# rongzhao-zhang/EfficientQ

Measured on AMD Instinct MI355X. Metric: ptq_calibration_throughput, higher is better.
Workload: dtype i8xi8->i32 (exact) for the Gram systems and per-iteration loss convs of the layers with quantised input, f32/f64 elsewhere

## Files before the change

### efficientq_amd/_lib.py

```python
from __future__ import annotations

import ctypes as C
import os

import torch

_HERE = os.path.dirname(os.path.abspath(__file__))
LIB_PATH = os.path.join(_HERE, "libeffq_hip.so")

EFFQ_OK = 0
_ERR_NAMES = {1: "EFFQ_ERR_ARG", 2: "EFFQ_ERR_HIP", 3: "EFFQ_ERR_WORKSPACE", 4: "EFFQ_ERR_NO_DEVICE",
              5: "EFFQ_ERR_NOT_CONVERGED"}


class EffqError(RuntimeError):
    pass


class Geom(C.Structure):
    _fields_ = [(n, C.c_int32) for n in
                ("N", "C1", "C2", "D", "H", "W", "KD", "KH", "KW", "SD", "SH", "SW", "PD", "PH", "PW")]

    def out_dims(self):
        return ((self.D + 2 * self.PD - self.KD) // self.SD + 1,
# ... 27 lines not shown
                ("ainv_pool", C.c_void_p), ("n_ainv", C.c_int32),
                ("prox_ws", C.c_void_p), ("prox_ws_bytes", C.c_size_t),
                ("red_ws", C.c_void_p),
                ("fp_ws", C.c_void_p), ("fp_ws_bytes", C.c_size_t),
                ("fp_pred", C.c_void_p), ("fp_traj_ws", C.c_void_p), ("fp_traj_ws_bytes", C.c_size_t),
                ("inv_ws", C.c_void_p), ("inv_ws_bytes", C.c_size_t),
                ("inv_ws_side", C.c_void_p), ("inv_ws_side_bytes", C.c_size_t),
                ("conv_ws", C.c_void_p), ("conv_ws_bytes", C.c_size_t),
                ("stream_main", C.c_void_p), ("stream_loss", C.c_void_p), ("stream_side", C.c_void_p),
                ("stream_side2", C.c_void_p), ("inv_ws_side2", C.c_void_p), ("inv_ws_side2_bytes", C.c_size_t),
                ("loss_Au", C.c_void_p), ("loss_Bu", C.c_void_p), ("loss_syy", C.c_void_p),
                ("loss_planes", C.c_void_p), ("loss_nplanes", C.c_int32), ("res_ring", C.c_void_p),
                ("channel_wise", C.c_int32), ("alpha_ring", C.c_void_p), ("w_iters_ring", C.c_void_p)]


class ProfRecord(C.Structure):
    _fields_ = [("kind", C.c_int32), ("iter", C.c_int32), ("loss_kind", C.c_int32), ("c2", C.c_int32), ("n", C.c_int32),
                ("geom", Geom), ("ms", C.c_float)]


SIGNATURES = {
    "effq_last_error": (C.c_char_p, []),
    "effq_version": (_I, []),
    "effq_device_count": (_I, [C.POINTER(C.c_int)]),
    "effq_quant_dequant_f32": (_I, [_P, _P, _F, _F, _I, _P, _P, _SZ, _P]),
    "effq_quant_dequant_f64path": (_I, [_P, _P, _D, _D, _I, _P, _P, _P, _SZ, _P]),
    "effq_reduce_ws_bytes": (_SZ, []),
    "effq_abs_sum_f64": (_I, [_P, _SZ, _P, _P, _P]),
    "effq_moments_f64": (_I, [_P, _SZ, _P, _P, _P]),
    "effq_alpha_stats_f64": (_I, [_P, _P, _D, _D, _I, _SZ, _P, _P, _P, _P]),
    "effq_fp_init": (_I, [_P, _P, _P]),
    "effq_fp_update": (_I, [_P, _D, _I, _P]),
    "effq_alpha_fixed_point": (_I, [_P, _SZ, _I, _D, _D, _D, _I, _I, _P, _P, _P]),
    "effq_fp_small_max": (_SZ, []),
    "effq_fixed_point_small": (_I, [_P, _P, _P, _SZ, _I, _D, _D, _D, _I, _P, _P]),
    "effq_fp_coop_max": (_SZ, []),
    "effq_fp_coop_set_spin_limit": (_I, [C.c_uint]),
    "effq_fixed_point_coop": (_I, [_P, _P, _P, _SZ, _I, _D, _D, _D, _I, _P, _P, _P]),
    "effq_fp_bucket_max": (_SZ, []),
    "effq_fp_bucket_ws_bytes": (_SZ, [_SZ]),
    "effq_fixed_point_bucket": (_I, [_P, _P, _P, _SZ, _I, _D, _D, _D, _I, _P, _P, _SZ, _P]),
    "effq_fp_bracket_ws_bytes": (_SZ, [_SZ]),
    "effq_fp_bracket_init": (_I, [_P, _P, _SZ, _I, _I, _P, _SZ, _P]),
    "effq_fp_bracket_run": (_I, [_P, _SZ, _I, _D, _D, _D, _I, _I, _P, _P, _P]),
    "effq_fp_bracket_stats": (_I, [_P, _SZ, _I, _D, _D, _P, _P, _P]),
    "effq_fp_bracket_update": (_I, [_SZ, _I, _D, _D, _D, _I, _P, _P, _P]),
    "effq_fp_traj_max": (_SZ, []),
    "effq_fp_traj_ws_bytes": (_SZ, [_SZ]),
    "effq_spd_inverse_prepare": (_I, [_P]),
    "effq_fp_traj_pred_bytes": (_SZ, []),
    "effq_fixed_point_traj": (_I, [_P, _P, _P, _SZ, _I, _D, _D, _D, _I, _P, _P, _P, _SZ, _P]),
    "effq_fixed_point_bucket_rec": (_I, [_P, _P, _P, _SZ, _I, _D, _D, _D, _I, _P, _P, _SZ, _P, _P]),
    "effq_fixed_point_coop_rec": (_I, [_P, _P, _P, _SZ, _I, _D, _D, _D, _I, _P, _P, _P, _P]),
    "effq_fp_check": (_I, [_P, _P, _P]),
    "effq_fp_channels_max_row": (_I, []),
    "effq_fixed_point_channels": (_I, [_P, _P, _P, _I, _I, _I, _D, _I, _P, _P, _P, _P]),
    "effq_fixed_point_channels_proj": (_I, [_P, _P, _P, _I, _I, _I, _D, _I, _P, _P, _P, _P, _F, _P, _P, _P, _I, _I, _D,
                                            _D, _P]),
    "effq_gram_packed_elems": (_SZ, [_I, _I]),
    "effq_gram_pack": (_I, [_P, _P, _I, _I, _P, _P]),
    "effq_gram_unpack": (_I, [_P, _I, _I, _P, _P, _P]),
    "effq_act_quant_backward": (_I, [_P, _P, _I, _P, _P, _P, _SZ, _P, _P]),
    "effq_att_classes_ws_bytes": (_SZ, []),
    "effq_att_classes": (_I, [_P, _LL, _P, _P, _P, C.POINTER(C.c_int32), _P, _P]),
    "effq_prof_enable": (_I, [_I]),
    "effq_prof_count": (_I, []),
    "effq_prof_read": (_I, [_I, C.POINTER(ProfRecord)]),
    "effq_admm_num_inverses": (_I, [_D, _D, _I, _I]),
    "effq_admm_run": (_I, [C.POINTER(AdmmRunArgs)]),
    "effq_admm_select_best": (_I, [_P, _I, _P, _P, _SZ, _SZ, _P, _P, _P, _P]),
    "effq_gram_ws_bytes": (_SZ, [_GP, _I]),
    "effq_gram_accum": (_I, [_P, _P, _P, _GP, _I, _P, _P, _I, _P, _SZ, _P]),
    "effq_gram_plan_query": (_I, [_GP, _I, _IP, _IP, _IP, _IP, _LLP, _IP, _IP]),
    "effq_gram_i8_supported": (_I, [_GP, _I]),
    "effq_gram_i8_ws_bytes": (_SZ, [_GP, _I]),
    "effq_gram_accum_i8": (_I, [_P, _P, _GP, _I, _P, _I, _P, _P, _P, _I, _LL, _P, _P, _I, _P, _SZ, _P]),
    "effq_gram_accum_i8_unw": (_I, [_P, _P, _GP, _I, _P, _I, _P, _P, _P, _I, _LL, _P, _P, _I, _P, _P, _P, _SZ, _P]),
    "effq_gram_i8_plan_query": (_I, [_GP, _I, _LL, _IP, _IP, _IP, _IP, _IP, _IP]),
    "effq_upsample_trilinear": (_I, [_P, _I, _I, _I, _I, _I, _I, _I, _I, _P, _P]),
    "effq_gram_f64_supported": (_I, [_GP, _I]),
    "effq_gram_f64_ws_bytes": (_SZ, [_GP, _I]),
    "effq_gram_f64": (_I, [_P, _P, _GP, _I, _P, _P, _P, _SZ, _P]),
    "effq_gram_f64_plan_query": (_I, [_GP, _I, _IP, _IP, _IP, _IP]),
    "effq_gram_loss_ws_bytes": (_SZ, [_I]),
    "effq_gram_loss": (_I, [_P, _P, _P, _P, _P, _I, _I, _I, _P, _P, _SZ, _P]),
    "effq_packed_bytes": (_SZ, [_SZ, _I]),
    "effq_pack_levels": (_I, [_P, _SZ, _I, _P, _P]),
    "effq_unpack_levels": (_I, [_P, _SZ, _I, _P, _P]),
    "effq_ainv_ld": (_I, [_I]),
    "effq_fp_bracket_export_words": (_SZ, []),
    "effq_fp_bracket_export": (_I, [_P, _SZ, _P, _P, _SZ, _P]),
    "effq_fp_bracket_rebase": (_I, [_P, _P, _SZ, _P]),
    "effq_fp_bracket_import": (_I, [_P, _SZ, _P, _I, _SZ, _P, _P, _SZ, _P]),
    "effq_admm_uses_traj": (_I, [_SZ, _I]),
    "effq_gram_loss_i8_supported": (_I, [_I, _I, _I, _I]),
    "effq_gram_loss_i8_num_planes": (_I, [C.c_longlong]),
    "effq_gram_loss_i8_planes_bytes": (_SZ, [_I, _I, _I]),
    "effq_gram_loss_i8_prepare": (_I, [_P, _I, _I, _P, _I, _I, _P, _P, _P]),
    "effq_gram_loss_i8_ws_bytes": (_SZ, []),
    "effq_gram_loss_i8": (_I, [_P, _I, _P, _P, _P, _P, _P, _P, _P, _I, _I, _I, _I, _I, _I, _P, _P, _SZ, _P]),
    "effq_spd_inverse_ws_bytes": (_SZ, [_I]),
    "effq_spd_inverse": (_I, [_P, _I, _I, _D, _D, _P, _P, _SZ, _P]),
    "effq_spd_inverse_plan": (_I, [_I, _IP, _IP, _IP]),
    "effq_prox_plan_query": (_I, [_I, _I, _IP, _IP, _IP, _IP]),
    "effq_prox_ws_bytes": (_SZ, [_I, _I]),
    "effq_prox_solve": (_I, [_P, _P, _P, _P, _P, _P, _I, _I, _I, _D, _D, _P, _P, _P, _SZ, _P]),
    "effq_prox_solve_shifted": (_I, [_P, _P, _P, _P, _P, _P, _I, _I, _I, _D, _D, _D, _I, _P, _P, _P, _SZ, _P]),
    "effq_admm_presum": (_I, [_P, _P, _P, _SZ, _P]),
    "effq_admm_project_dual": (_I, [_P, _P, _P, _I, _P, _P, _F, _P, _SZ, _P]),
    "effq_conv_plan_query": (_I, [_GP, _I, _IP, _IP, _IP, _IP, _IP, _IP, _IP, _IP, _LLP]),
    "effq_conv_i8_plan_query": (_I, [_GP, _I, _IP, _IP, _IP, _IP]),
    "effq_conv_i8s_plan_query": (_I, [_GP, _I, _I, _IP, _IP, _IP, _IP, _IP, _IP, _IP]),
    "effq_conv_i8_supported": (_I, [_GP, _I, _I]),
    "effq_conv_i8s_supported": (_I, [_GP, _I, _I]),
    "effq_conv_i8s_ws_bytes": (_SZ, [_GP, _I, _I]),
    "conv3d_calib_step_i8s": (_I, [_P, _P, _P, _P, _GP, _P, _I, _P, _I, _I, _P, _P, _SZ, _P]),
    "effq_conv_i8_ws_bytes": (_SZ, [_GP]),
    "conv3d_calib_step_i8": (_I, [_P, _P, _P, _P, _GP, _P, _I, _P, _I, _P, _P, _SZ, _P]),
    "effq_conv_i8_out_supported": (_I, [_GP, _I, _I]),
    "conv3d_quant_forward_i8": (_I, [_P, _P, _P, _P, _P, _GP, _P, _I, _P, _I, _P, _P, _P, _SZ, _P]),
    "effq_conv_ws_bytes": (_SZ, [_GP]),
    "conv3d_quant_calib_step": (_I, [_P, _P, _P, _P, _P, _GP, _P, _I, _P, _P, _P, _SZ, _P]),
    "effq_adam_step": (_I, [_P, _P, _P, _P, _D, _D, _D, _D, _I, _SZ, _P]),
    "effq_window_gather": (_I, [_P, _I, _I, _I, _I, _I, _I, _I, _I, _I, _I, _I, _I, _I, _I, _P, _P]),
    "effq_window_put": (_I, [_P, _I, _I, _I, _I, _I, _I, _I, _P, _P]),
    "effq_window_stitch": (_I, [_P, _I, _I, _I, _I, _I, _I, _I, _I, _I, _I, _I, _P, _P, _P, _I, _P, _P]),
    "effq_seg_tallies": (_I, [_P, _P, _I, _LL, _I, _I, _F, _P, _P, _SZ, _P]),
    "effq_seg_sweep": (_I, [_P, _P, _I, _LL, _I, _I, _F, _P, _P]),
    "effq_seg_sweep_edges": (_I, [_I, _F, _P]),
    "effq_seg_sweep_plan": (_I, [_I, _LL, _I, _IP, _IP]),
    "effq_seg_labels": (_I, [_P, _I, _I, _LL, _I, _I, _F, _I, _P, _P]),
    "effq_seg_labels_source": (_I, [_P, _I, _P, _P, _P, _P, _P, _I, _I, _F, _P, _P]),
    "effq_seg_probs_source": (_I, [_P, _I, _P, _P, _P, _P, _P, _I, _P, _P, _P]),
    "effq_seg_agreement": (_I, [_P, _P, _I, _LL, _I, _I, _F, _P, _P, _P, _P, _P, _SZ, _P]),
    "effq_cc_ws_bytes": (_SZ, [_I, _I, _I, _I]),
    "effq_cc_label": (_I, [_P, _I, _I, _I, _I, _I, _P, _P, _P, _SZ, _P]),
    "effq_seg_lesions": (_I, [_P, _P, _I, _I, _I, _I, _I, _I, _F, _I, _P, _P, _SZ, _P]),
    "effq_cc_table_ws_bytes": (_SZ, [_I, _I, _I, _I, _I]),
    "effq_cc_table": (_I, [_P, _I, _I, _I, _I, _I, _I, _P, _P, _P, _SZ, _P]),
    "effq_seg_lesion_table": (_I, [_P, _P, _I, _I, _I, _I, _I, _I, _F, _I, _I, _P, _P, _P, _P, _SZ, _P]),
    "effq_label_clean_ws_bytes": (_SZ, [_I, _I, _I]),
    "effq_label_clean": (_I, [_P, _I, _I, _I, _I, _I, _P, _P, _P, _P, _P, _SZ, _P]),
    "effq_label_tallies_ws_bytes": (_SZ, []),
    "effq_label_tallies": (_I, [_P, _P, _I, _I, _LL, _P, _P, _P, _SZ, _P]),
    "effq_surf_ws_bytes": (_SZ, [_I, _I, _I, _I]),
    "effq_edt_sq": (_I, [_P, _I, _I, _I, _I, _P, _P, _SZ, _P]),
    "effq_seg_surface": (_I, [_P, _P, _I, _I, _I, _I, _I, _I, _F, _P, _P, _P, _SZ, _P]),
    "effq_surf_mm_ws_bytes": (_SZ, [_I, _I, _I, _I]),
    "effq_edt_sq_mm": (_I, [_P, _I, _I, _I, _I, _F, _F, _F, _P, _P, _SZ, _P]),
    "effq_seg_surface_mm": (_I, [_P, _P, _I, _I, _I, _I, _I, _I, _F, _F, _F, _F, _P, _P, _P, _P, _SZ, _P]),
    "effq_prep_window": (_I, [_P, _SZ, _F, _F, _P]),
    "effq_prep_resample": (_I, [_P, _I, _I, _I, _I, _D, _D, _D, _I, _P, _I, _I, _I, _P]),
    "effq_prep_bbox_moments": (_I, [_P, _I, _I, _I, _I, _I, _P, _P, _P, _P, _SZ, _P]),
    "effq_prep_sqdev": (_I, [_P, _I, _LL, _I, _P, _P, _P, _SZ, _P]),
    "effq_prep_standardise_crop": (_I, [_P, _I, _I, _I, _I, _I, _P, _P, _P, _P, _P, _P]),
    "effq_prep_crop_u8": (_I, [_P, _I, _I, _I, _I, _P, _P, _P, _P]),
    "effq_prep_union_mask": (_I, [_P, _I, _LL, _I, _P, _P]),
    "effq_prep_reorient": (_I, [_P, _I, _I, _I, _I, _P, _I, _I, _P, _P]),
    "effq_prep_reorient_plan": (_I, [_P, _I, _I, _P]),
}

SEG_TALLIES_WS_BYTES = 1024 * 3 * 8 * 4
SEG_TALLIES_MAX_CLASSES = 8
SEG_AGREEMENT_WS_BYTES = 768 * (4 * SEG_TALLIES_MAX_CLASSES * 8 + (3 * SEG_TALLIES_MAX_CLASSES + 1) * 4)
SEG_ARGMAX, SEG_SIGMOID = 0, 1
SEG_SWEEP_BINS = 4096
# ... 37 lines not shown
```

### efficientq_amd/csrc/gram_f64.hip

```cpp
#include "common.h"

namespace effq {

typedef double f64x4g __attribute__((ext_vector_type(4)));

constexpr int GF_VC = 32;
constexpr int GF_T = 256;
constexpr int GF_MAXN = 128, GF_MAXC2 = 64;
constexpr int GF_MAXTILES = 72;

struct GramF64Params {
  const float* x;
  const float* y;
  effq_geom g;
  int n, has_bias, np, c2p, ld;
  int od, oh, ow;
  long long V;
  int nchunk, ntiles, te, tc;
  double* slab;
};

template <int TPW>
__global__ __launch_bounds__(GF_T, (TPW <= 6) ? 4 : 2) void k_gram_f64(GramF64Params p) {
  extern __shared__ __attribute__((aligned(16))) double rows[];
  __shared__ int tab_a[GF_MAXTILES], tab_b[GF_MAXTILES];
  const int tid = threadIdx.x, lane = tid & 63, wid = tid >> 6;
  const int lr = lane & 15, lk = lane >> 4;
  if (tid == 0) {
    int t = 0;
    for (int i = 0; i < p.te; ++i)
      for (int j = i; j < p.te; ++j) {
        tab_a[t] = 16 * i;
        tab_b[t] = 16 * j;
        ++t;
      }
    for (int c = 0; c < p.tc; ++c)
      for (int j = 0; j < p.te; ++j) {
        tab_a[t] = p.np + 16 * c;
        tab_b[t] = 16 * j;
        ++t;
      }
  }
  __syncthreads();
  int aoff[TPW], boff[TPW];
  f64x4g acc[TPW];
#pragma unroll
  for (int t = 0; t < TPW; ++t) {
    const int tile = wid + 4 * t;
    const bool ok = tile < p.ntiles;
    aoff[t] = ok ? tab_a[tile] : 0;
    boff[t] = ok ? tab_b[tile] : 0;
#pragma unroll
    for (int r = 0; r < 4; ++r) acc[t][r] = 0.0;
  }
  const int nw = p.n - p.has_bias;
  __shared__ int qtab[GF_MAXN];
  __shared__ int vrow[GF_VC][4];
  {
    const int k3 = p.g.KD * p.g.KH * p.g.KW, k2 = p.g.KH * p.g.KW;
    for (int q = tid; q < nw; q += GF_T) {
      const int c = q / k3, kr = q - c * k3;
      const int kd = kr / k2, kr2 = kr - kd * k2;
      const int kh = kr2 / p.g.KW, kw = kr2 - kh * p.g.KW;
      qtab[q] = c | (kd << 16) | (kh << 20) | (kw << 24);
    }
  }
  const int rowlen = p.np + p.c2p;
  const int V = (int)p.V;
  for (int ch = blockIdx.x; ch < p.nchunk; ch += gridDim.x) {
    __syncthreads();
    const int v0 = ch * GF_VC;
    if (tid < GF_VC) {
      const int v = v0 + tid;
      int t = v;
      const int ow_ = t % p.ow;
      t /= p.ow;
      const int oh_ = t % p.oh;
      t /= p.oh;
      const int od_ = t % p.od;
      vrow[tid][0] = (v < V) ? t / p.od : -1;
      vrow[tid][1] = od_ * p.g.SD - p.g.PD;
      vrow[tid][2] = oh_ * p.g.SH - p.g.PH;
      vrow[tid][3] = ow_ * p.g.SW - p.g.PW;
    }
    __syncthreads();
    for (int e = tid; e < GF_VC * rowlen; e += GF_T) {
      const int vl = e / rowlen, q = e - vl * rowlen;
      const int nn = vrow[vl][0];
      double val = 0.0;
      if (nn >= 0) {
        if (q < nw) {
          const int pk = qtab[q];
          const int c = pk & 0xffff;
          const int id = vrow[vl][1] + ((pk >> 16) & 15), ih = vrow[vl][2] + ((pk >> 20) & 15),
                    iw = vrow[vl][3] + ((pk >> 24) & 15);
          if (id >= 0 && id < p.g.D && ih >= 0 && ih < p.g.H && iw >= 0 && iw < p.g.W)
            val = (double)p.x[((((size_t)nn * p.g.D + id) * p.g.H + ih) * p.g.W + iw) * p.g.C1 + c];
        } else if (q < p.n) {
          val = 1.0;
        } else if (q >= p.np && q - p.np < p.g.C2) {
          val = (double)p.y[(size_t)(v0 + vl) * p.g.C2 + (q - p.np)];
        }
      }
      rows[vl * p.ld + q] = val;
    }
    __syncthreads();
#pragma unroll 2
    for (int ks = 0; ks < GF_VC / 4; ++ks) {
      const double* r0 = rows + (ks * 4 + lk) * p.ld + lr;
#pragma unroll
      for (int t = 0; t < TPW; ++t) {
        const double a = r0[aoff[t]], b = r0[boff[t]];
        acc[t] = __builtin_amdgcn_mfma_f64_16x16x4f64(a, b, acc[t], 0, 0, 0);
      }
    }
  }
#pragma unroll
  for (int t = 0; t < TPW; ++t) {
    const int tile = wid + 4 * t;
    if (tile < p.ntiles) {
      double* dst = p.slab + ((size_t)blockIdx.x * p.ntiles + tile) * 256;
#pragma unroll
      for (int r = 0; r < 4; ++r) dst[r * 64 + lane] = acc[t][r];
    }
  }
}

__global__ __launch_bounds__(256) void k_gram_f64_reduce(GramF64Params p, int nslab, double* __restrict__ Au,
                                                         double* __restrict__ Bu) {
  const int tile = blockIdx.x, e = threadIdx.x;
  double s = 0.0;
  for (int w = 0; w < nslab; ++w) s += p.slab[((size_t)w * p.ntiles + tile) * 256 + e];
  const int r = e >> 6, lane = e & 63;
  const int row = (lane >> 4) + 4 * r, col = lane & 15;
  const int nau = p.te * (p.te + 1) / 2;
  if (tile < nau) {
    int i = 0, rem = tile;
    while (rem >= p.te - i) {
      rem -= p.te - i;
      ++i;
    }
    const int j = i + rem;
    const int gi = 16 * i + row, gj = 16 * j + col;
    if (gi < p.n && gj < p.n) {
      Au[(size_t)gi * p.n + gj] = s;
      if (i != j) Au[(size_t)gj * p.n + gi] = s;
    }
  } else {
    const int t = tile - nau;
    const int c = t / p.te, j = t - c * p.te;
    const int gc = 16 * c + row, gj = 16 * j + col;
    if (gc < p.g.C2 && gj < p.n) Bu[(size_t)gc * p.n + gj] = s;
  }
}

static bool gram_f64_plan(const effq_geom* g, int has_bias, GramF64Params* p) {
  if (g == nullptr) return false;
  const long long nw = (long long)g->C1 * g->KD * g->KH * g->KW;
  const long long n = nw + (has_bias ? 1 : 0);
  if (n < 1 || n > GF_MAXN || g->C2 < 1 || g->C2 > GF_MAXC2) return false;
  const int od = (g->D + 2 * g->PD - g->KD) / g->SD + 1, oh = (g->H + 2 * g->PH - g->KH) / g->SH + 1,
            ow = (g->W + 2 * g->PW - g->KW) / g->SW + 1;
  if (od <= 0 || oh <= 0 || ow <= 0 || g->N <= 0) return false;
  p->g = *g;
  p->n = (int)n;
  p->has_bias = has_bias ? 1 : 0;
  p->np = ((int)n + 15) / 16 * 16;
  p->c2p = (g->C2 + 15) / 16 * 16;
  p->ld = p->np + p->c2p + 2;
  p->od = od; p->oh = oh; p->ow = ow;
  p->V = (long long)g->N * od * oh * ow;
  p->nchunk = (int)((p->V + GF_VC - 1) / GF_VC);
  p->te = p->np / 16;
  p->tc = p->c2p / 16;
  p->ntiles = p->te * (p->te + 1) / 2 + p->tc * p->te;
  return p->ntiles <= GF_MAXTILES && p->V < ((long long)1 << 31) - GF_VC && g->KD <= 15 && g->KH <= 15 && g->KW <= 15;
}

static int gram_f64_grid(const GramF64Params& p) { return p.nchunk < 1024 ? p.nchunk : 1024; }

static int gram_f64_tpw(const GramF64Params& p) {
  const int tpw = (p.ntiles + 3) / 4;
  return tpw <= 3 ? 3 : (tpw <= 6 ? 6 : (tpw <= 11 ? 11 : 18));
}

}
using namespace effq;

extern "C" {

int effq_gram_f64_supported(const effq_geom* g, int has_bias) {
  GramF64Params p;
  return gram_f64_plan(g, has_bias, &p) ? 1 : 0;
}

size_t effq_gram_f64_ws_bytes(const effq_geom* g, int has_bias) {
  GramF64Params p;
  if (!gram_f64_plan(g, has_bias, &p)) return 0;
  return (size_t)gram_f64_grid(p) * p.ntiles * 256 * sizeof(double);
}

int effq_gram_f64(const float* x_ndhwc, const float* y_ndhwc, const effq_geom* g, int has_bias, double* Au, double* Bu,
                  void* ws, size_t ws_bytes, void* stream) {
  EFFQ_CHECK_ARG(x_ndhwc && y_ndhwc && g && Au && Bu && ws);
  GramF64Params p;
  if (!gram_f64_plan(g, has_bias, &p)) {
    set_error("gram_f64: unsupported geometry (n = C1*k^3 + bias <= %d, C2 <= %d)", GF_MAXN, GF_MAXC2);
    return EFFQ_ERR_ARG;
  }
  const size_t need = effq_gram_f64_ws_bytes(g, has_bias);
  if (ws_bytes < need) {
    set_error("gram_f64: workspace %zu < required %zu", ws_bytes, need);
    return EFFQ_ERR_WORKSPACE;
  }
  p.x = x_ndhwc;
  p.y = y_ndhwc;
  p.slab = reinterpret_cast<double*>(ws);
  const int grid = gram_f64_grid(p);
  const size_t lds = (size_t)GF_VC * p.ld * sizeof(double);
  hipStream_t st = as_stream(stream);
#define EFFQ_GF(TPW_) hipLaunchKernelGGL((k_gram_f64<TPW_>), dim3(grid), dim3(GF_T), lds, st, p)
  switch (gram_f64_tpw(p)) {
    case 3: EFFQ_GF(3); break;
    case 6: EFFQ_GF(6); break;
    case 11: EFFQ_GF(11); break;
    default: EFFQ_GF(18); break;
  }
#undef EFFQ_GF
  EFFQ_LAUNCH_CHECK();
  hipLaunchKernelGGL(k_gram_f64_reduce, dim3(p.ntiles), dim3(256), 0, st, p, grid, Au, Bu);
  EFFQ_LAUNCH_CHECK();
  return EFFQ_OK;
}

int effq_gram_f64_plan_query(const effq_geom* g, int has_bias, int* nchunk, int* grid, int* ntiles, int* tpw) {
  EFFQ_CHECK_ARG(g && nchunk && grid && ntiles && tpw);
  GramF64Params p;
  EFFQ_CHECK_ARG(gram_f64_plan(g, has_bias, &p));
  *nchunk = p.nchunk;
  *grid = gram_f64_grid(p);
  *ntiles = p.ntiles;
  *tpw = gram_f64_tpw(p);
  return EFFQ_OK;
}

}
```

### efficientq_amd/hip_ops.py

```python
from __future__ import annotations

import ctypes as C
import math
from typing import Optional, Tuple

import torch

from . import _lib
from ._lib import Geom, check

ADMM_TOL = 1e-5
FP_BRACKET_MIN = 1 << 18
DP_GATHER_AFTER = 4
DP_GATHER_MAX_BYTES = 128 << 20


def _ptr(t: Optional[torch.Tensor]):
    return None if t is None else C.c_void_p(t.data_ptr())


def to_ndhwc(x: torch.Tensor) -> torch.Tensor:
    return x.permute(0, 2, 3, 4, 1).contiguous()


# ... 379 lines not shown
        check(self.lib.effq_gram_plan_query(C.byref(geom), int(has_bias), C.byref(vec), C.byref(nb), C.byref(npairs),
                                            C.byref(nsplit), C.byref(vps), C.byref(fold), C.byref(fin)),
              "effq_gram_plan_query")
        return dict(vec=bool(vec.value), NB=nb.value, npairs=npairs.value, nsplit=nsplit.value, vox_per_split=vps.value,
                    fold=fold.value, finish_blocks=fin.value)

    def gram_i8_plan(self, geom: Geom, ncls: int = 1, n_list: int = 0) -> dict:
        out = [C.c_int() for _ in range(6)]
        check(self.lib.effq_gram_i8_plan_query(C.byref(geom), int(ncls), int(n_list), *[C.byref(o) for o in out]),
              "effq_gram_i8_plan_query")
        return dict(zip(("NB", "NBX", "npairs", "nchunks", "cps", "nsplit"), (o.value for o in out)))

    def gram_f64_plan(self, geom: Geom, has_bias: bool) -> dict:
        out = [C.c_int() for _ in range(4)]
        check(self.lib.effq_gram_f64_plan_query(C.byref(geom), int(has_bias), *[C.byref(o) for o in out]),
              "effq_gram_f64_plan_query")
        return dict(zip(("nchunk", "grid", "ntiles", "tpw"), (o.value for o in out)))

    def gram_i8_supported(self, geom: Geom, act_levels: int) -> bool:
        return bool(self.lib.effq_gram_i8_supported(C.byref(geom), int(act_levels)))

    GRAM_I8_MAX_CLASSES = 16

    def att_classes(self, att: Optional[torch.Tensor]):
        if att is None:
            return (None, None, None, 1)
        key = (att.data_ptr(), att.numel(), att._version)
        hit = self._att_cache.get(key)
        if hit is not None:
            return hit[1]
        flat = self._f32(att).reshape(-1)
        V = flat.numel()
        lst = torch.empty(V + 128 * self.GRAM_I8_MAX_CLASSES, dtype=torch.int32, device=flat.device)
        chunk_cls = torch.empty(V // 128 + self.GRAM_I8_MAX_CLASSES, dtype=torch.int32, device=flat.device)
        cls_w = torch.empty(self.GRAM_I8_MAX_CLASSES, dtype=torch.float32, device=flat.device)
        info = (C.c_int32 * 3)()
        ws = self._workspace("att_cls", self.lib.effq_att_classes_ws_bytes())
        check(self.lib.effq_att_classes(_ptr(flat), V, _ptr(lst), _ptr(chunk_cls), _ptr(cls_w), info, _ptr(ws),
                                        self.stream), "effq_att_classes")
        k, n_list, overflow = int(info[0]), int(info[1]), int(info[2])
        res = None if overflow else (lst[:n_list], chunk_cls[: n_list // 128], cls_w[:k], k)
        if len(self._att_cache) > 16:
            self._att_cache.clear()
        self._att_cache[key] = (att, res)
        return res

    def gram_i8(self, xidx_ndhwc: torch.Tensor, att_cls, y_ndhwc: torch.Tensor, geom: Geom, has_bias: bool,
                act_alpha: torch.Tensor, act_levels: int, A0: Optional[torch.Tensor] = None,
                B0: Optional[torch.Tensor] = None, unweighted: bool = False):
        if xidx_ndhwc.dtype != torch.uint8 or not xidx_ndhwc.is_contiguous():
            raise _lib.EffqError("gram_i8 wants contiguous uint8 level ids")
        y = self._f32(y_ndhwc)
        _check_shapes(geom, xidx_ndhwc, y=y)
        lst, chunk_cls, cls_w, ncls = att_cls
        if lst is not None:
            od, oh, ow = geom.out_dims()
            if (int(lst.numel()) < geom.N * od * oh * ow or lst.numel() % 128 or
                    chunk_cls.numel() * 128 != lst.numel() or cls_w.numel() != ncls):
                raise _lib.EffqError("gram_i8: voxel list does not match the output volume")
        n = geom.C1 * geom.KD * geom.KH * geom.KW + int(has_bias)
        acc = int(A0 is not None)
        if A0 is not None and (tuple(A0.shape) != (n, n) or tuple(B0.shape) != (geom.C2, n)):
            raise _lib.EffqError("gram_i8: A0/B0 shapes do not match the geometry")
        if A0 is None:
            A0 = torch.empty(n, n, dtype=torch.float32, device=self.device)
            B0 = torch.empty(geom.C2, n, dtype=torch.float32, device=self.device)
        al = self._f32(act_alpha.reshape(1))
        ws = self._workspace("gram_i8", self.lib.effq_gram_i8_ws_bytes(C.byref(geom), int(ncls)))
        Au = Bu = None
        if unweighted:
            if acc:
                raise _lib.EffqError("gram_i8: the unweighted system is not accumulated across calls here")
            Au = torch.empty(n, n, dtype=torch.float64, device=self.device)
            Bu = torch.empty(geom.C2, n, dtype=torch.float64, device=self.device)
        check(self.lib.effq_gram_accum_i8_unw(_ptr(xidx_ndhwc), _ptr(y), C.byref(geom), int(has_bias), _ptr(al),
                                              int(act_levels), _ptr(lst), _ptr(chunk_cls), _ptr(cls_w), int(ncls),
                                              0 if lst is None else int(lst.numel()), _ptr(A0), _ptr(B0), acc,
                                              _ptr(Au), _ptr(Bu), _ptr(ws), ws.numel(), self.stream),
              "effq_gram_accum_i8_unw")
        return (A0, B0, Au, Bu) if unweighted else (A0, B0)

    def gram_f64_supported(self, geom: Geom, has_bias: bool) -> bool:
        return bool(self.lib.effq_gram_f64_supported(C.byref(geom), int(has_bias)))

    def gram_f64(self, x_ndhwc: torch.Tensor, y_ndhwc: torch.Tensor, geom: Geom, has_bias: bool):
        x, y = self._f32(x_ndhwc), self._f32(y_ndhwc)
        _check_shapes(geom, x, y=y)
        n = geom.C1 * geom.KD * geom.KH * geom.KW + int(has_bias)
        Au = torch.empty(n, n, dtype=torch.float64, device=self.device)
        Bu = torch.empty(geom.C2, n, dtype=torch.float64, device=self.device)
        ws = self._workspace("gram_f64", self.lib.effq_gram_f64_ws_bytes(C.byref(geom), int(has_bias)))
        check(self.lib.effq_gram_f64(_ptr(x), _ptr(y), C.byref(geom), int(has_bias), _ptr(Au), _ptr(Bu), _ptr(ws),
                                     ws.numel(), self.stream), "effq_gram_f64")
        return Au, Bu

    def upsample_trilinear(self, x_ndhwc: torch.Tensor, scale) -> torch.Tensor:
        x = self._f32(x_ndhwc)
        N, D, H, W, Cc = (int(i) for i in x.shape)
        sd, sh, sw = (int(i) for i in scale)
        out = torch.empty(N, D * sd, H * sh, W * sw, Cc, dtype=torch.float32, device=self.device)
        check(self.lib.effq_upsample_trilinear(_ptr(x), N, D, H, W, Cc, sd, sh, sw, _ptr(out), self.stream),
              "effq_upsample_trilinear")
        return out

    def gram_loss(self, Au: torch.Tensor, Bu: torch.Tensor, syy: torch.Tensor, G: torch.Tensor, b, sqerr=None):
        c2, n = (int(i) for i in Bu.shape)
        has_b = b is not None
        if (Au.dtype != torch.float64 or Bu.dtype != torch.float64 or syy.dtype != torch.float64 or
                tuple(Au.shape) != (n, n) or G.numel() != c2 * (n - int(has_b))):
            raise _lib.EffqError("gram_loss: operand shapes / dtypes do not match")
        if sqerr is None:
            sqerr = torch.zeros(2, dtype=torch.float64, device=self.device)
        ws = self._workspace("gram_loss", self.lib.effq_gram_loss_ws_bytes(n))
        check(self.lib.effq_gram_loss(_ptr(Au), _ptr(Bu), _ptr(syy), _ptr(self._f32(G)), _ptr(b), c2, n, int(has_b),
                                      _ptr(sqerr), _ptr(ws), ws.numel(), self.stream), "effq_gram_loss")
        return sqerr

    def gram_loss_i8_supported(self, c2: int, n: int, has_b: bool, w_levels: int) -> bool:
        return bool(self.lib.effq_gram_loss_i8_supported(int(c2), int(n), int(has_b), int(w_levels)))

    def gram_loss_i8_planes(self, Au: torch.Tensor, has_b: bool, act_alpha: torch.Tensor, act_levels: int, voxels: int):
        n = int(Au.shape[0])
        P = self.lib.effq_gram_loss_i8_num_planes(int((act_levels - 1) ** 2 * voxels))
        if P < 1:
            return None
        nw = n - int(has_b)
        planes = torch.empty(P, (nw + 255) // 256 * 256, nw, dtype=torch.int8, device=self.device)
        assert planes.numel() == self.lib.effq_gram_loss_i8_planes_bytes(n, int(has_b), P)
        err = torch.zeros(1, dtype=torch.int32, device=self.device)
        al = self._f32(act_alpha.reshape(1))
        check(self.lib.effq_gram_loss_i8_prepare(_ptr(Au), n, int(has_b), _ptr(al), int(act_levels), P, _ptr(planes),
                                                 _ptr(err), self.stream), "effq_gram_loss_i8_prepare")
        planes._effq_err = err
        return planes

    def gram_loss_i8(self, planes, Au, Bu, syy, Gq, b, states, act_alpha, act_levels: int, w_levels: int, hist=None):
        count, c2 = int(Gq.shape[0]), int(Bu.shape[0])
        n = int(Bu.shape[1])
        has_b = b is not None
        if hist is None:
            hist = torch.zeros(count, 2, dtype=torch.float64, device=self.device)
        ws = self._workspace("gram_loss_i8", self.lib.effq_gram_loss_i8_ws_bytes())
        al = self._f32(act_alpha.reshape(1))
        check(self.lib.effq_gram_loss_i8(_ptr(planes), int(planes.shape[0]), _ptr(Au), _ptr(Bu), _ptr(syy), _ptr(Gq), _ptr(b),
                                         _ptr(states), _ptr(al), int(act_levels), int(w_levels), c2, n, int(has_b), count,
                                         _ptr(hist), _ptr(ws), ws.numel(), self.stream), "effq_gram_loss_i8")
        return hist

    def gram_reduce(self, A0: torch.Tensor, B0: torch.Tensor, reducer):
        n, c2 = int(A0.shape[0]), int(B0.shape[0])
        buf = torch.empty(self.lib.effq_gram_packed_elems(n, c2), dtype=torch.float32, device=self.device)
        check(self.lib.effq_gram_pack(_ptr(A0), _ptr(B0), n, c2, _ptr(buf), self.stream), "effq_gram_pack")
        reducer(buf)
        check(self.lib.effq_gram_unpack(_ptr(buf), n, c2, _ptr(A0), _ptr(B0), self.stream), "effq_gram_unpack")
        return A0, B0

    @staticmethod
    def storage_bits(levels: int) -> int:
        for b in (1, 2, 4, 8):
            if levels <= (1 << b):
                return b
        raise _lib.EffqError(f"{levels} levels do not fit 8 bits")

    def pack_levels(self, idx: torch.Tensor, bits: int) -> torch.Tensor:
        if idx.dtype != torch.uint8 or not idx.is_contiguous():
            raise _lib.EffqError("pack_levels wants contiguous uint8 level ids")
# ... 1000 lines not shown
```

### include/effq_hip.h

```cpp
#ifndef EFFQ_HIP_H
#define EFFQ_HIP_H

#include <stddef.h>
#include <stdint.h>

#ifdef __cplusplus
extern "C" {
#endif

enum {
  EFFQ_OK = 0,
  EFFQ_ERR_ARG = 1,
  EFFQ_ERR_HIP = 2,
  EFFQ_ERR_WORKSPACE = 3,
  EFFQ_ERR_NO_DEVICE = 4,
  EFFQ_ERR_NOT_CONVERGED = 5
};

typedef struct effq_geom {
  int32_t N, C1, C2;
  int32_t D, H, W;
  int32_t KD, KH, KW;
  int32_t SD, SH, SW;
  int32_t PD, PH, PW;
// ... 26 lines not shown
  int32_t done;
} effq_fp_state;

int effq_fp_init(effq_fp_state* state_dev, const double* abs_sums_dev, void* stream);
int effq_fp_update(effq_fp_state* state_dev, double tol, int max_iter, void* stream);

int effq_alpha_fixed_point(const float* x, size_t n, int levels, double lo, double hi, double tol,
                           int max_iter, int n_iters, effq_fp_state* state_dev, void* ws, void* stream);

size_t effq_fp_small_max(void);
int effq_fixed_point_small(const float* a, const float* b, float* v_out, size_t n, int levels, double lo, double hi,
                           double tol, int max_iter, effq_fp_state* state_dev, void* stream);
size_t effq_fp_coop_max(void);
int effq_fixed_point_coop(const float* a, const float* b, float* v_out, size_t n, int levels, double lo, double hi,
                          double tol, int max_iter, effq_fp_state* state_dev, void* ws, void* stream);
int effq_fp_coop_set_spin_limit(unsigned int polls);
size_t effq_fp_bucket_max(void);
size_t effq_fp_bucket_ws_bytes(size_t n);
int effq_fixed_point_bucket(const float* a, const float* b, float* v_out, size_t n, int levels, double lo, double hi,
                            double tol, int max_iter, effq_fp_state* state_dev, void* ws, size_t ws_bytes,
                            void* stream);

size_t effq_fp_traj_max(void);
size_t effq_fp_traj_ws_bytes(size_t n);
size_t effq_fp_traj_pred_bytes(void);
int effq_fixed_point_traj(const float* a, const float* b, float* v_out, size_t n, int levels, double lo, double hi,
                          double tol, int max_iter, effq_fp_state* state_dev, void* pred_dev, void* ws, size_t ws_bytes,
                          void* stream);
int effq_fixed_point_bucket_rec(const float* a, const float* b, float* v_out, size_t n, int levels, double lo, double hi,
                                double tol, int max_iter, effq_fp_state* state_dev, void* ws, size_t ws_bytes,
                                void* pred_dev, void* stream);
int effq_fixed_point_coop_rec(const float* a, const float* b, float* v_out, size_t n, int levels, double lo, double hi,
                              double tol, int max_iter, effq_fp_state* state_dev, void* ws, void* pred_dev, void* stream);

size_t effq_fp_bracket_ws_bytes(size_t n);
int effq_fp_bracket_init(effq_fp_state* state_dev, const double* abs_sums_dev, size_t n, int levels, int list_first,
                         void* ws, size_t ws_bytes, void* stream);
int effq_fp_bracket_run(const float* x, size_t n, int levels, double lo, double hi, double tol, int max_iter, int n_iters,
                        effq_fp_state* state_dev, void* ws, void* stream);
int effq_fp_bracket_stats(const float* x, size_t n, int levels, double lo, double hi, effq_fp_state* state_dev, void* ws,
                          void* stream);
int effq_fp_bracket_update(size_t n, int levels, double lo, double hi, double tol, int max_iter,
                           effq_fp_state* state_dev, void* ws, void* stream);
size_t effq_fp_bracket_export_words(void);
int effq_fp_bracket_export(const void* ws, size_t n, long long* out, float* list_out, size_t list_cap, void* stream);
int effq_fp_bracket_import(const void* ws_src, size_t n_src, const long long* pack_dev, int world, size_t list_cap,
                           effq_fp_state* state_dev, void* ws_dst, size_t ws_dst_bytes, void* stream);
int effq_fp_bracket_rebase(effq_fp_state* state_dev, void* ws, size_t n, void* stream);
int effq_fp_channels_max_row(void);
int effq_fixed_point_channels(const float* a, const float* b, float* v_out, int c2, int nwrow, int levels, double tol,
                              int max_iter, double* alpha_out, int32_t* iters_out, int32_t* err_flag_dev, void* stream);
int effq_fixed_point_channels_proj(const float* wstar, float* dual, float* v_out, int c2, int nwrow, int levels,
                                   double tol, int max_iter, double* alpha_out, int32_t* iters_out, int32_t* err_flag_dev,
                                   float* G, float dual_div, float* Bm, const float* B0, const float* W0, int n, int ldb,
                                   double rho_next, double eta, void* stream);

int effq_fp_check(const effq_fp_state* state_dev, int32_t* err_flag_dev, void* stream);

size_t effq_gram_ws_bytes(const effq_geom* g, int has_bias);
int effq_gram_accum(const float* x_ndhwc, const float* att, const float* y_ndhwc, const effq_geom* g,
                    int has_bias, float* A0, float* B0, int accumulate, void* ws, size_t ws_bytes,
                    void* stream);
int effq_gram_plan_query(const effq_geom* g, int has_bias, int* vec, int* nb, int* npairs, int* nsplit,
                         long long* vox_per_split, int* fold, int* finish_blocks);

int effq_gram_i8_supported(const effq_geom* g, int act_levels);
size_t effq_gram_i8_ws_bytes(const effq_geom* g, int ncls);
int effq_gram_accum_i8(const uint8_t* xidx_ndhwc, const float* y_ndhwc, const effq_geom* g, int has_bias,
                       const float* act_alpha_dev, int act_levels, const int32_t* vox_list,
                       const int32_t* chunk_cls, const float* cls_w_dev, int ncls, long long n_list,
                       float* A0, float* B0, int accumulate, void* ws, size_t ws_bytes, void* stream);
int effq_gram_accum_i8_unw(const uint8_t* xidx_ndhwc, const float* y_ndhwc, const effq_geom* g, int has_bias,
                           const float* act_alpha_dev, int act_levels, const int32_t* vox_list, const int32_t* chunk_cls,
                           const float* cls_w_dev, int ncls, long long n_list, float* A0, float* B0, int accumulate,
                           double* Au, double* Bu, void* ws, size_t ws_bytes, void* stream);
int effq_gram_i8_plan_query(const effq_geom* g, int ncls, long long n_list, int* nb, int* nbx, int* npairs, int* nchunks,
                            int* cps, int* nsplit);

int effq_gram_f64_supported(const effq_geom* g, int has_bias);
size_t effq_gram_f64_ws_bytes(const effq_geom* g, int has_bias);
int effq_gram_f64(const float* x_ndhwc, const float* y_ndhwc, const effq_geom* g, int has_bias, double* Au, double* Bu,
                  void* ws, size_t ws_bytes, void* stream);
int effq_gram_f64_plan_query(const effq_geom* g, int has_bias, int* nchunk, int* grid, int* ntiles, int* tpw);

size_t effq_gram_loss_ws_bytes(int n);
int effq_gram_loss(const double* Au, const double* Bu, const double* syy_dev, const float* G, const float* b, int c2, int n,
                   int has_bias, double* sqerr_out, void* ws, size_t ws_bytes, void* stream);

int effq_gram_loss_i8_supported(int c2, int n, int has_bias, int w_levels);
int effq_gram_loss_i8_num_planes(long long kmax);
size_t effq_gram_loss_i8_planes_bytes(int n, int has_bias, int nplanes);
int effq_gram_loss_i8_prepare(const double* Au, int n, int has_bias, const float* act_alpha_dev, int act_levels,
                              int nplanes, int8_t* planes, int32_t* err_flag_dev, void* stream);
size_t effq_gram_loss_i8_ws_bytes(void);
int effq_gram_loss_i8(const int8_t* planes, int nplanes, const double* Au, const double* Bu, const double* syy_dev,
                      const int8_t* Gq, const float* b, const effq_fp_state* states, const float* act_alpha_dev,
                      int act_levels, int w_levels, int c2, int n, int has_bias, int count, double* hist_out, void* ws,
                      size_t ws_bytes, void* stream);


size_t effq_att_classes_ws_bytes(void);
int effq_att_classes(const float* att, long long V, int32_t* vox_list, int32_t* chunk_cls, float* cls_w_dev,
                     int32_t* info_host_out, void* ws, void* stream);

int effq_spd_inverse_prepare(void* stream);
int effq_ainv_ld(int n);
size_t effq_spd_inverse_ws_bytes(int n);
int effq_spd_inverse(const float* A0, int n, int has_bias, double rho, double eta, float* Ainv,
                     void* ws, size_t ws_bytes, void* stream);
int effq_spd_inverse_plan(int n, int* wide, int* nblk, int* pivot_blocks);

size_t effq_prox_ws_bytes(int c2, int n);
int effq_prox_solve(const float* B0, const float* Ainv, const float* W0, const float* b0, const float* G,
                    const float* dual, int c2, int n, int has_bias, double rho, double eta, float* wstar,
                    float* bstar, void* ws, size_t ws_bytes, void* stream);
int effq_prox_plan_query(int c2, int n, int* variant, int* gx, int* gy, int* nsplit);

int effq_prox_solve_shifted(const float* B0, const float* Ainv, const float* W0, const float* b0, const float* G,
                            const float* dual, int c2, int n, int has_bias, double rho, double eta,
                            double rho_inv, int nterms, float* wstar, float* bstar, void* ws, size_t ws_bytes,
                            void* stream);

int effq_admm_presum(const float* wstar, const float* dual, float* v, size_t n, void* stream);
int effq_admm_project_dual(const float* v, const float* wstar, const effq_fp_state* state_dev, int levels,
                           float* G, float* dual, float dual_div, int8_t* Gq_out, size_t n, void* stream);
size_t effq_conv_ws_bytes(const effq_geom* g);
int conv3d_quant_calib_step(const float* xq_ndhwc, const float* G, const float* bias, const float* y_fp,
                            const float* att, const effq_geom* g, const float* act_alpha_dev, int act_levels,
                            double* sqerr_out, float* out, void* ws, size_t ws_bytes, void* stream);
int effq_conv_plan_query(const effq_geom* g, int loss_only, int* kind, int* fast, int* cslab, int* nslab, int* nt,
                         int* grid_x, int* grid_y, int* ntiles, long long* lds_bytes);

int effq_conv_i8_supported(const effq_geom* g, int act_levels, int w_levels);
size_t effq_conv_i8_ws_bytes(const effq_geom* g);
int conv3d_calib_step_i8(const uint8_t* xidx_ndhwc, const int8_t* Gq, const float* bias, const float* y_fp,
                         const effq_geom* g, const float* act_alpha_dev, int act_levels,
                         const effq_fp_state* w_state_dev, int w_levels, double* sqerr_out, void* ws,
                         size_t ws_bytes, void* stream);
int effq_conv_i8_out_supported(const effq_geom* g, int act_levels, int w_levels);
int conv3d_quant_forward_i8(const uint8_t* xidx_ndhwc, const int8_t* Gq, const float* bias, const float* y_fp,
                            const float* att, const effq_geom* g, const float* act_alpha_dev, int act_levels,
                            const effq_fp_state* w_state_dev, int w_levels, double* sqerr_out, float* out, void* ws,
                            size_t ws_bytes, void* stream);
int effq_conv_i8_plan_query(const effq_geom* g, int want_out, int* kernel, int* grid_x, int* grid_y, int* ntiles);

int effq_conv_i8s_supported(const effq_geom* g, int act_levels, int w_levels);
size_t effq_conv_i8s_ws_bytes(const effq_geom* g, int act_levels, int w_levels);
int conv3d_calib_step_i8s(const uint8_t* xidx_ndhwc, const int8_t* Gq, const float* bias, const float* y_fp,
                          const effq_geom* g, const float* act_alpha_dev, int act_levels,
                          const effq_fp_state* w_state_dev, int w_levels, int prepare, double* sqerr_out,
                          void* ws, size_t ws_bytes, void* stream);
int effq_conv_i8s_plan_query(const effq_geom* g, int act_levels, int w_levels, int* nj, int* ct, int* taps, int* k,
                             int* aoff, int* wmul, int* grid);

int effq_act_quant_backward(const float* x, const float* alpha_dev, int levels, const float* gq, float* gx_out,
                            double* galpha_out, size_t n, void* ws, void* stream);
int effq_adam_step(float* p, const float* g, float* m, float* v, double lr, double b1, double b2, double eps,
                   int t, size_t n, void* stream);

typedef struct effq_admm_run_args {
  const float* A0; const float* B0; const float* W0; const float* b0;
  int32_t c2, n, has_bias, w_levels;
  int32_t iters, rho_period;
  double rho, rho_max, eta, tol;
  effq_geom geom;
  int32_t loss_kind, act_levels;
// ... 149 lines not shown
```

Baseline: 24.78.

## Software-pipeline f64 Gram kernel with register prefetch and vectorised im2col staging

```diff
diff --git a/efficientq_amd/_lib.py b/efficientq_amd/_lib.py
--- a/efficientq_amd/_lib.py
+++ b/efficientq_amd/_lib.py
@@ -133,6 +133,7 @@
     "effq_gram_f64_ws_bytes": (_SZ, [_GP, _I]),
     "effq_gram_f64": (_I, [_P, _P, _GP, _I, _P, _P, _P, _SZ, _P]),
     "effq_gram_f64_plan_query": (_I, [_GP, _I, _IP, _IP, _IP, _IP]),
+    "effq_gram_f64_pipelined": (_I, [_P, _P, _GP, _I]),
     "effq_gram_loss_ws_bytes": (_SZ, [_I]),
     "effq_gram_loss": (_I, [_P, _P, _P, _P, _P, _I, _I, _I, _P, _P, _SZ, _P]),
     "effq_packed_bytes": (_SZ, [_SZ, _I]),
diff --git a/efficientq_amd/csrc/gram_f64.hip b/efficientq_amd/csrc/gram_f64.hip
--- a/efficientq_amd/csrc/gram_f64.hip
+++ b/efficientq_amd/csrc/gram_f64.hip
@@ -8,6 +8,7 @@
 constexpr int GF_T = 256;
 constexpr int GF_MAXN = 128, GF_MAXC2 = 64;
 constexpr int GF_MAXTILES = 72;
+constexpr int GF_NX = 4;
 
 struct GramF64Params {
   const float* x;
@@ -18,10 +19,12 @@
   long long V;
   int nchunk, ntiles, te, tc;
   double* slab;
+  int vecy;
+  int step[4];
 };
 
-template <int TPW>
-__global__ __launch_bounds__(GF_T, (TPW <= 6) ? 4 : 2) void k_gram_f64(GramF64Params p) {
+template <int TPW, bool PIPE>
+__global__ __launch_bounds__(GF_T, (TPW <= 3 || (TPW <= 6 && !PIPE)) ? 4 : 2) void k_gram_f64(GramF64Params p) {
   extern __shared__ __attribute__((aligned(16))) double rows[];
   __shared__ int tab_a[GF_MAXTILES], tab_b[GF_MAXTILES];
   const int tid = threadIdx.x, lane = tid & 63, wid = tid >> 6;
@@ -54,10 +57,24 @@
     for (int r = 0; r < 4; ++r) acc[t][r] = 0.0;
   }
   const int nw = p.n - p.has_bias;
+  const int k3 = p.g.KD * p.g.KH * p.g.KW, k2 = p.g.KH * p.g.KW;
+  const int V = (int)p.V;
+  constexpr int KUNROLL = PIPE ? 1 : 2;
+  auto consume = [&]() {
+#pragma unroll KUNROLL
+    for (int ks = 0; ks < GF_VC / 4; ++ks) {
+      const double* r0 = rows + (ks * 4 + lk) * p.ld + lr;
+#pragma unroll
+      for (int t = 0; t < TPW; ++t) {
+        const double a = r0[aoff[t]], b = r0[boff[t]];
+        acc[t] = __builtin_amdgcn_mfma_f64_16x16x4f64(a, b, acc[t], 0, 0, 0);
+      }
+    }
+  };
+  if constexpr (!PIPE) {
   __shared__ int qtab[GF_MAXN];
   __shared__ int vrow[GF_VC][4];
   {
-    const int k3 = p.g.KD * p.g.KH * p.g.KW, k2 = p.g.KH * p.g.KW;
     for (int q = tid; q < nw; q += GF_T) {
       const int c = q / k3, kr = q - c * k3;
       const int kd = kr / k2, kr2 = kr - kd * k2;
@@ -66,7 +83,6 @@
     }
   }
   const int rowlen = p.np + p.c2p;
-  const int V = (int)p.V;
   for (int ch = blockIdx.x; ch < p.nchunk; ch += gridDim.x) {
     __syncthreads();
     const int v0 = ch * GF_VC;
@@ -105,15 +121,107 @@
       rows[vl * p.ld + q] = val;
     }
     __syncthreads();
-#pragma unroll 2
-    for (int ks = 0; ks < GF_VC / 4; ++ks) {
-      const double* r0 = rows + (ks * 4 + lk) * p.ld + lr;
-#pragma unroll
-      for (int t = 0; t < TPW; ++t) {
-        const double a = r0[aoff[t]], b = r0[boff[t]];
-        acc[t] = __builtin_amdgcn_mfma_f64_16x16x4f64(a, b, acc[t], 0, 0, 0);
-      }
-    }
+    consume();
+  }
+  } else {
+  const int c4x = p.g.C1 >> 2, perx = k3 * c4x, nx = GF_VC * perx;
+  const int ycell = p.vecy ? (p.g.C2 >> 2) : p.g.C2, ny = GF_VC * ycell;
+  const int ncell = (nx + GF_T - 1) / GF_T;
+  int xkd[GF_NX], xkh[GF_NX], xkw[GF_NX], xc[GF_NX], xd[GF_NX];
+  int vn[GF_NX], vd[GF_NX], vh[GF_NX], vw[GF_NX];
+  float4 px[GF_NX], py = make_float4(0.f, 0.f, 0.f, 0.f);
+  bool okx[GF_NX], oky = false;
+#pragma unroll
+  for (int i = 0; i < GF_NX; ++i) {
+    const int e = min(tid + i * GF_T, nx - 1);
+    const int vl = e / perx, r = e - vl * perx;
+    const int tap = r / c4x, c4 = r - tap * c4x;
+    const int kd = tap / k2, kr2 = tap - kd * k2, kh = kr2 / p.g.KW;
+    xkd[i] = kd - p.g.PD;
+    xkh[i] = kh - p.g.PH;
+    xkw[i] = kr2 - kh * p.g.KW - p.g.PW;
+    xc[i] = 4 * c4;
+    xd[i] = vl * p.ld + 4 * c4 * k3 + tap;
+    int t = blockIdx.x * GF_VC + vl;
+    vw[i] = t % p.ow;
+    t /= p.ow;
+    vh[i] = t % p.oh;
+    t /= p.oh;
+    vd[i] = t % p.od;
+    vn[i] = t / p.od;
+    px[i] = make_float4(0.f, 0.f, 0.f, 0.f);
+    okx[i] = false;
+  }
+  const int ye = min(tid, ny - 1), yl = ye / ycell, yc = (ye - yl * ycell) * (p.vecy ? 4 : 1);
+  auto prefetch = [&](int ch) {
+#pragma unroll
+    for (int i = 0; i < GF_NX; ++i)
+      if (i < ncell) {
+        const int id = vd[i] * p.g.SD + xkd[i], ih = vh[i] * p.g.SH + xkh[i], iw = vw[i] * p.g.SW + xkw[i];
+        okx[i] = vn[i] < p.g.N && id >= 0 && id < p.g.D && ih >= 0 && ih < p.g.H && iw >= 0 && iw < p.g.W;
+        const int cn = min(vn[i], p.g.N - 1), cd = min(max(id, 0), p.g.D - 1), chh = min(max(ih, 0), p.g.H - 1),
+                  cw = min(max(iw, 0), p.g.W - 1);
+        px[i] = *reinterpret_cast<const float4*>(
+            p.x + ((((size_t)cn * p.g.D + cd) * p.g.H + chh) * p.g.W + cw) * p.g.C1 + xc[i]);
+        int c;
+        vw[i] += p.step[3];
+        c = vw[i] >= p.ow;
+        vw[i] -= c ? p.ow : 0;
+        vh[i] += p.step[2] + c;
+        c = vh[i] >= p.oh;
+        vh[i] -= c ? p.oh : 0;
+        vd[i] += p.step[1] + c;
+        c = vd[i] >= p.od;
+        vd[i] -= c ? p.od : 0;
+        vn[i] = min(vn[i] + p.step[0] + c, p.g.N);
+      }
+    const int v = ch * GF_VC + yl;
+    oky = v < V;
+    const float* src = p.y + (size_t)(oky ? v : 0) * p.g.C2 + yc;
+    if (p.vecy)
+      py = *reinterpret_cast<const float4*>(src);
+    else
+      py.x = *src;
+  };
+  {
+    const int t0 = p.np - p.n, trest = t0 + p.c2p - p.g.C2;
+    for (int e = tid; e < GF_VC * trest; e += GF_T) {
+      const int vl = e / trest, r = e - vl * trest;
+      rows[vl * p.ld + (r < t0 ? p.n + r : p.np + p.g.C2 + (r - t0))] = 0.0;
+    }
+  }
+  auto stage = [&](int ch) {
+#pragma unroll
+    for (int i = 0; i < GF_NX; ++i)
+      if (tid + i * GF_T < nx) {
+        const float4 val = okx[i] ? px[i] : make_float4(0.f, 0.f, 0.f, 0.f);
+        double* d = rows + xd[i];
+        d[0] = (double)val.x;
+        d[k3] = (double)val.y;
+        d[2 * k3] = (double)val.z;
+        d[3 * k3] = (double)val.w;
+      }
+    if (tid < ny) {
+      const float4 val = oky ? py : make_float4(0.f, 0.f, 0.f, 0.f);
+      double* d = rows + yl * p.ld + p.np + yc;
+      d[0] = (double)val.x;
+      if (p.vecy) {
+        d[1] = (double)val.y;
+        d[2] = (double)val.z;
+        d[3] = (double)val.w;
+      }
+    }
+    if (p.has_bias && tid < GF_VC) rows[tid * p.ld + nw] = (ch * GF_VC + tid < V) ? 1.0 : 0.0;
+  };
+  prefetch(blockIdx.x);
+  for (int ch = blockIdx.x; ch < p.nchunk; ch += gridDim.x) {
+    __syncthreads();
+    stage(ch);
+    __syncthreads();
+    const int next = ch + gridDim.x;
+    prefetch(next < p.nchunk ? next : ch);
+    consume();
+  }
   }
 #pragma unroll
   for (int t = 0; t < TPW; ++t) {
@@ -129,8 +237,18 @@
 __global__ __launch_bounds__(256) void k_gram_f64_reduce(GramF64Params p, int nslab, double* __restrict__ Au,
                                                          double* __restrict__ Bu) {
   const int tile = blockIdx.x, e = threadIdx.x;
+  const double* src = p.slab + (size_t)tile * 256 + e;
+  const size_t stride = (size_t)p.ntiles * 256;
   double s = 0.0;
-  for (int w = 0; w < nslab; ++w) s += p.slab[((size_t)w * p.ntiles + tile) * 256 + e];
+  int w = 0;
+  for (; w + 16 <= nslab; w += 16) {
+    double v[16];
+#pragma unroll
+    for (int k = 0; k < 16; ++k) v[k] = src[(size_t)(w + k) * stride];
+#pragma unroll
+    for (int k = 0; k < 16; ++k) s += v[k];
+  }
+  for (; w < nslab; ++w) s += src[(size_t)w * stride];
   const int r = e >> 6, lane = e & 63;
   const int row = (lane >> 4) + 4 * r, col = lane & 15;
   const int nau = p.te * (p.te + 1) / 2;
@@ -184,6 +302,14 @@
   return tpw <= 3 ? 3 : (tpw <= 6 ? 6 : (tpw <= 11 ? 11 : 18));
 }
 
+static bool gram_f64_pipe(const GramF64Params& p, const void* x, const void* y, int* vecy) {
+  const effq_geom& g = p.g;
+  if ((g.C1 & 3) != 0 || (reinterpret_cast<uintptr_t>(x) & 15) != 0) return false;
+  *vecy = ((g.C2 & 3) == 0 && (reinterpret_cast<uintptr_t>(y) & 15) == 0) ? 1 : 0;
+  const int xcells = GF_VC * (p.n - p.has_bias) / 4, ycells = GF_VC * (*vecy ? g.C2 / 4 : g.C2);
+  return xcells <= GF_NX * GF_T && ycells <= GF_T && gram_f64_tpw(p) <= 11;
+}
+
 }
 using namespace effq;
 
@@ -219,12 +345,23 @@
   const int grid = gram_f64_grid(p);
   const size_t lds = (size_t)GF_VC * p.ld * sizeof(double);
   hipStream_t st = as_stream(stream);
-#define EFFQ_GF(TPW_) hipLaunchKernelGGL((k_gram_f64<TPW_>), dim3(grid), dim3(GF_T), lds, st, p)
+  p.vecy = 0;
+  const bool pipe = gram_f64_pipe(p, x_ndhwc, y_ndhwc, &p.vecy);
+  {
+    long long t = (long long)grid * GF_VC;
+    p.step[3] = (int)(t % p.ow);
+    t /= p.ow;
+    p.step[2] = (int)(t % p.oh);
+    t /= p.oh;
+    p.step[1] = (int)(t % p.od);
+    p.step[0] = (int)(t / p.od);
+  }
+#define EFFQ_GF(TPW_, PIPE_) hipLaunchKernelGGL((k_gram_f64<TPW_, PIPE_>), dim3(grid), dim3(GF_T), lds, st, p)
   switch (gram_f64_tpw(p)) {
-    case 3: EFFQ_GF(3); break;
-    case 6: EFFQ_GF(6); break;
-    case 11: EFFQ_GF(11); break;
-    default: EFFQ_GF(18); break;
+    case 3: if (pipe) EFFQ_GF(3, true); else EFFQ_GF(3, false); break;
+    case 6: if (pipe) EFFQ_GF(6, true); else EFFQ_GF(6, false); break;
+    case 11: if (pipe) EFFQ_GF(11, true); else EFFQ_GF(11, false); break;
+    default: EFFQ_GF(18, false); break;
   }
 #undef EFFQ_GF
   EFFQ_LAUNCH_CHECK();
@@ -244,4 +381,10 @@
   return EFFQ_OK;
 }
 
-}
+int effq_gram_f64_pipelined(const float* x_ndhwc, const float* y_ndhwc, const effq_geom* g, int has_bias) {
+  GramF64Params p;
+  int vecy = 0;
+  return (gram_f64_plan(g, has_bias, &p) && gram_f64_pipe(p, x_ndhwc, y_ndhwc, &vecy)) ? 1 : 0;
+}
+
+}
diff --git a/efficientq_amd/hip_ops.py b/efficientq_amd/hip_ops.py
--- a/efficientq_amd/hip_ops.py
+++ b/efficientq_amd/hip_ops.py
@@ -485,6 +485,9 @@
 
     def gram_f64_supported(self, geom: Geom, has_bias: bool) -> bool:
         return bool(self.lib.effq_gram_f64_supported(C.byref(geom), int(has_bias)))
+
+    def gram_f64_pipelined(self, x_ndhwc: torch.Tensor, y_ndhwc: torch.Tensor, geom: Geom, has_bias: bool) -> bool:
+        return bool(self.lib.effq_gram_f64_pipelined(_ptr(x_ndhwc), _ptr(y_ndhwc), C.byref(geom), int(has_bias)))
 
     def gram_f64(self, x_ndhwc: torch.Tensor, y_ndhwc: torch.Tensor, geom: Geom, has_bias: bool):
         x, y = self._f32(x_ndhwc), self._f32(y_ndhwc)
diff --git a/include/effq_hip.h b/include/effq_hip.h
--- a/include/effq_hip.h
+++ b/include/effq_hip.h
@@ -132,6 +132,7 @@
 int effq_gram_f64(const float* x_ndhwc, const float* y_ndhwc, const effq_geom* g, int has_bias, double* Au, double* Bu,
                   void* ws, size_t ws_bytes, void* stream);
 int effq_gram_f64_plan_query(const effq_geom* g, int has_bias, int* nchunk, int* grid, int* ntiles, int* tpw);
+int effq_gram_f64_pipelined(const float* x_ndhwc, const float* y_ndhwc, const effq_geom* g, int has_bias);
 
 size_t effq_gram_loss_ws_bytes(int n);
 int effq_gram_loss(const double* Au, const double* Bu, const double* syy_dev, const float* G, const float* b, int c2, int n,
```

After: 25.15 (median of 6 runs). 1.5% higher.
